# THU-luvision/TextureFusion

Hardware: AMD Instinct MI355X
Metric: RGB-D frames/s (TSDF integrate + atlas update: prepare->integrate->finalize, UpdateMeshes, GeneratePatches + UpdateAtlas over the frame's dirty chunks) (higher is better)
Workload: dtype f32

## Files before the change

texturefusion_amd/csrc/tf_mesh.hip:

```cpp
#include <stdlib.h>
#include <string.h>

#include <algorithm>
#include <vector>

#include "tf_devfn.h"
#include "tf_kf_store.h"
#include "tf_mc_table.h"
#include "tf_patch_body.h"
#include "tf_volume.h"

#pragma clang fp contract(off)

namespace tf {

__device__ const unsigned long long d_mc_tri[256] = TF_MC_TRI_TABLE_INIT;

constexpr int kR = 11;
constexpr int kRS = 11;
constexpr int kPS = kRS * kR;
constexpr int kRV = kPS * kR;
constexpr int kEdgeSlots = 3 * 729;
__device__ __forceinline__ uint32_t mesh_shard_rows_d(uint32_t max_chunks) { return max_chunks / kMeshShards + 258u; }

__device__ __forceinline__ int ridx(int x, int y, int z) { return (x + 1) + (y + 1) * kRS + (z + 1) * kPS; }

constexpr bool halo_needed(int rx, int ry, int rz) {
  if (rx < -1 || rx > 9 || ry < -1 || ry > 9 || rz < -1 || rz > 9) return false;
  if (rx >= 0 && rx < 8 && ry >= 0 && ry < 8 && rz >= 0 && rz < 8) return false;
  const int out = ((rx < 0 || rx > 8) ? 1 : 0) + ((ry < 0 || ry > 8) ? 1 : 0) + ((rz < 0 || rz > 8) ? 1 : 0);
  return out <= 1;
}
constexpr int count_halo_pairs() {
  int n = 0;
  for (int rz = -1; rz <= 9; ++rz)
    for (int ry = -1; ry <= 9; ++ry)
      for (int rx = -1; rx <= 9; ++rx) {
        if (!halo_needed(rx, ry, rz)) continue;
        const int vx = (rx + 8) & 7;
        if ((vx & 1) && halo_needed(rx - 1, ry, rz) && (((rx - 1 + 8) >> 3) == ((rx + 8) >> 3))) continue;
        ++n;
      }
  return n;
}
constexpr int kHalo = count_halo_pairs();
struct MeshTabs {
  unsigned long long halo[kHalo];
  uint16_t corner[729];
};
constexpr unsigned long long corner_of(int rx, int ry, int rz) {
  return (rx >= 0 && ry >= 0 && rz >= 0 && rx <= 8 && ry <= 8 && rz <= 8) ? (unsigned long long)(rx + ry * 9 + rz * 81 + 1) : 0ull;
}
constexpr MeshTabs make_mesh_tabs() {
  MeshTabs t{};
  int n = 0;
  for (int rz = -1; rz <= 9; ++rz)
    for (int ry = -1; ry <= 9; ++ry)
      for (int rx = -1; rx <= 9; ++rx) {
        if (!halo_needed(rx, ry, rz)) continue;
        const int vx = (rx + 8) & 7;
        const bool same_chunk_left = ((rx - 1 + 8) >> 3) == ((rx + 8) >> 3);
        if ((vx & 1) && halo_needed(rx - 1, ry, rz) && same_chunk_left) continue;
        const int rx0 = (vx & 1) ? rx - 1 : rx;
        const bool use0 = !(vx & 1);
        const bool use1 = (vx & 1) ? true : (halo_needed(rx + 1, ry, rz) && (((rx + 1 + 8) >> 3) == ((rx + 8) >> 3)));
        const int cx = (rx + 8) >> 3, cy = (ry + 8) >> 3, cz = (rz + 8) >> 3;
        const unsigned long long nb = (unsigned long long)(cx + cy * 3 + cz * 9);
        const unsigned long long pair = (unsigned long long)((((rx0 + 8) & 7) + ((ry + 8) & 7) * 8 + ((rz + 8) & 7) * 64) >> 1);
        const unsigned long long r0 = (unsigned long long)((rx0 + 1) + (ry + 1) * kRS + (rz + 1) * kPS);
        t.halo[n++] = (r0 & 2047ull) | (nb << 11) | (pair << 16) | ((use0 ? 1ull : 0ull) << 24) | ((use1 ? 1ull : 0ull) << 25) |
                      ((use0 ? corner_of(rx0, ry, rz) : 0ull) << 26) | ((use1 ? corner_of(rx0 + 1, ry, rz) : 0ull) << 36);
      }
  for (int c = 0; c < 729; ++c) {
    const int px = c % 9, py = (c / 9) % 9, pz = c / 81;
    t.corner[c] = (uint16_t)((px + 1) + (py + 1) * kRS + (pz + 1) * kPS);
  }
  return t;
}
__device__ const MeshTabs d_mesh_tabs = make_mesh_tabs();

__device__ __forceinline__ int cox(int k) { return (0x66 >> k) & 1; }
__device__ __forceinline__ int coy(int k) { return (0xCC >> k) & 1; }
__device__ __forceinline__ int coz(int k) { return (0xF0 >> k) & 1; }
__device__ __forceinline__ int edge_c0(int e) { return (int)((0x321076543210ull >> (4 * e)) & 0xF); }
__device__ __forceinline__ int edge_c1(int e) { return (int)((0x765447650321ull >> (4 * e)) & 0xF); }

__device__ __forceinline__ int edge_slot(int x, int y, int z, int e) {
  const int bx = x + ((0x622 >> e) & 1);
  const int by = y + ((0xC44 >> e) & 1);
  const int bz = z + ((0x0F0 >> e) & 1);
  const int ax = e >= 8 ? 2 : (e & 1);
  return ax + (bx + by * 9 + bz * 81) * 3;
}
__device__ __forceinline__ int edge_of_slot(int ax, int dx, int dy, int dz) {
  if (ax == 0) return dz ? (dy ? 6 : 4) : (dy ? 2 : 0);
  if (ax == 1) return dz ? (dx ? 5 : 7) : (dx ? 1 : 3);
  return dy ? (dx ? 10 : 11) : (dx ? 9 : 8);
}

__device__ __forceinline__ bool gradient_at(const float* __restrict__ S, int px, int py, int pz, int ox, int oy,
                                            int oz, float res, float g[3]) {
  const int c = ridx(px, py, pz);
  const float xm = S[c - 1], xp = S[c + 1];
  const float ym = S[c - kRS], yp = S[c + kRS];
  const float zm = S[c - kPS], zp = S[c + kPS];
  const bool ok = ((ox ? xp : xm) < 1.0f) && ((oy ? yp : ym) < 1.0f) && ((oz ? zp : zm) < 1.0f);
  const float gx = xp - xm, gy = yp - ym, gz = zp - zm;
  const float yz = gy * gy + gz * gz;
  const float sq = gx * gx + yz;
  const float n = sqrtf(sq);
  g[0] = gx; g[1] = gy; g[2] = gz;
  if (sq > 0.0f) { g[0] = gx / n; g[1] = gy / n; g[2] = gz / n; }
  return ok && !(n > res * 100.0f);
}

constexpr uint32_t kCfHeavy = 64u;
constexpr uint32_t kCfGradOk = 128u;

template <int NT>
struct MeshSh {
  float S[kRV];
  uint8_t cflag[732];
  uint32_t nslot[27];
  unsigned long long rmask[NT];
  uint16_t rbase[NT];
  uint32_t ownq[(kEdgeSlots + 7) / 8];
  uint16_t cinfo[512];
  uint8_t cidx[512];
  uint16_t toff[512];
  uint32_t wsum[8];
  uint32_t nv, nt, adj, any;
  uint32_t ncell;
  uint16_t clist[512];
  uint32_t ovf;
  uint32_t rblock;
  uint32_t rpress;
  uint32_t rstate;
  unsigned long long rtexloc;
};

__device__ __forceinline__ int edge_q(int e) {
  return (int)((0x231023320110ull >> (4 * e)) & 0x3);
}
__device__ __forceinline__ int owner_cell(int m, int q) {
  const int ax = m % 3, b = m / 3;
  const int bx = b % 9, by = (b / 9) % 9, bz = b / 81;
  const int d0 = q & 1, d1 = q >> 1;
  int x, y, z;
  if (ax == 0) { x = bx; y = by - d0; z = bz - d1; }
  else if (ax == 1) { x = bx - d0; y = by; z = bz - d1; }
  else { x = bx - d0; y = by - d1; z = bz; }
  return x + 8 * y + 64 * z;
}

__device__ __forceinline__ void patch_list_append(const VolumeDev& v, int ppar, uint32_t shard, const int4 id,
                                                  uint32_t slot, unsigned long long texloc, uint32_t blk) {
  const uint32_t rows = mesh_shard_rows_d(v.max_chunks);
  const uint32_t p = atomicAdd(&v.patch_cnt[((ppar & 1) * kMeshShards + shard) * 16], 1u);
  const unsigned long long key = pack_id(id.x, id.y, id.z);
  if (p < rows) v.patch_list[((size_t)(ppar & 1) * kMeshShards + shard) * rows + p] = make_int4((int)(uint32_t)key, (int)(uint32_t)(key >> 32), (int)slot, (int)blk);
  else atomicOr(&v.vctl->status, kStMeshFull);
  if (texloc == kNoTexloc) {
    const uint32_t c = atomicAdd(&v.actl->set[ppar & 1].n_cand, 1u);
    if (c < v.max_chunks) v.cand[c] = pack_id(id.x, id.y, id.z);
  }
}

__device__ __forceinline__ void filter_reset_record(const VolumeDev& v, uint32_t own, const int4 id, uint32_t epoch, int ppar) {
  MeshRec* rec = &v.mesh_rec[own];
  const uint32_t was = rec->state;
  const uint32_t inmap = was & kMsInMap;
  rec->nv = 0; rec->nt = 0; rec->state = inmap | ((ppar >= 0 && inmap) ? kMsSimplified : 0u); rec->epoch = epoch;
  if (inmap) {
    uint32_t blk = rec->block;
    const unsigned long long texloc = rec->texloc;
    if (blk != kBlkNone && blk_pressed(blk_pressure(v), blk)) {
      blk_release(v, blk);
      rec->block = blk = kBlkNone;
    }
    if (ppar >= 0) patch_list_append(v, ppar, own & (kMeshShards - 1u), id, own, texloc, blk);
  }
}

__device__ __forceinline__ void filter_defer_reset(const VolumeDev& v, uint32_t* cnt, uint32_t cap_sh, uint32_t own, const int4 id) {
  const uint32_t shard = own & (kMeshShards - 1u);
  const uint32_t p = atomicAdd(&cnt[(2u * kMeshShards + shard) * 16u], 1u);
  if (p < cap_sh) v.reset_list[(size_t)shard * cap_sh + p] = make_int4(id.x, id.y, id.z, (int)own);
}

__device__ const uint8_t kFarWord[19] = {0, 1, 2, 3, 4, 5, 6, 7, 8, 9, 10, 11, 12, 15, 18, 19, 20, 21, 24};
__device__ __forceinline__ uint32_t filter_near(const VolumeDev& v, const int4 id, int lane, int k8, uint32_t own_in, bool listed,
                                                bool use_summ, uint32_t create_seq, uint32_t* own, bool* maybe) {
  uint32_t nslot = kInvalidSlot;
  *maybe = true;
  if (own_in != kInvalidSlot) {
    const int word = k8 == 0 ? kNbrStamp : 13 + (k8 & 1) + 3 * ((k8 >> 1) & 1) + 9 * (k8 >> 2);
    uint32_t w = v.nbr[(size_t)own_in * kNbrWords + word];
    uint32_t alive = 1u;
    if (k8 == 0 && listed && id.w > 0) alive = v.hent[(uint32_t)id.w - 1u].alive & 1u;
    const uint32_t st = (uint32_t)__shfl((int)w, lane & 56);
    if (!(st > create_seq)) {
      if (k8 != 0 && w == 0u) {
        w = nbr_probe(v, pack_id(id.x + (k8 & 1), id.y + ((k8 >> 1) & 1), id.z + (k8 >> 2)));
        if (w) v.nbr[(size_t)own_in * kNbrWords + word] = w;
      }
      for (int q = k8; q < 19; q += 8) {
        const int fw = (int)kFarWord[q];
        if (v.nbr[(size_t)own_in * kNbrWords + fw] == 0u) {
          const uint32_t got = nbr_probe(v, pack_id(id.x + fw % 3 - 1, id.y + (fw / 3) % 3 - 1, id.z + fw / 9 - 1));
          if (got) v.nbr[(size_t)own_in * kNbrWords + fw] = got;
        }
      }
      if (k8 == 0) v.nbr[(size_t)own_in * kNbrWords + kNbrStamp] = v.seq;
    }
    nslot = k8 == 0 ? (alive ? own_in : kInvalidSlot) : (w ? w - 1u : kInvalidSlot);
  }
  *own = (uint32_t)__shfl((int)nslot, lane & 56);
  if (use_summ && *own != kInvalidSlot) {
    const uint32_t sm = nslot != kInvalidSlot ? v.summ[nslot] : 0u;
    const uint32_t sel = k8 == 0 ? 0u : ((k8 & 1) ? 4u : ((k8 & 2) ? 8u : 12u));
    uint32_t u = (sm >> sel) & 15u;
    u |= (uint32_t)__shfl_xor((int)u, 1); u |= (uint32_t)__shfl_xor((int)u, 2); u |= (uint32_t)__shfl_xor((int)u, 4);
    const uint32_t so = (uint32_t)__shfl((int)sm, lane & 56);
    *maybe = (so & 1u) && (u & 14u) == 14u;
  }
  return nslot;
}

template <bool HAVE_ROW>
__device__ __forceinline__ void filter_exact(const VolumeDev& v, const int4 id, uint32_t nslot, const uint32_t own, int lane,
                                             uint32_t epoch, uint32_t* __restrict__ surv, uint32_t* __restrict__ cnt,
                                             uint32_t cap_sh, int ppar, bool use_summ, bool defer, uint32_t create_seq) {
  const uint32_t shard = own & (kMeshShards - 1u);
  const float4* T4 = reinterpret_cast<const float4*>(v.tsdf + (size_t)own * kChunkVoxels);
  uint32_t roww = 0u;
  if (!HAVE_ROW && lane < kNbrWords) roww = v.nbr[(size_t)own * kNbrWords + lane];
  float4 qv[4];
#pragma unroll
  for (int j = 0; j < 4; ++j) qv[j] = T4[j * 64 + lane];
  const uint32_t had_mesh = v.mesh_rec[own].state & kMsInMap;
  uint32_t fl = 0;
#pragma unroll
  for (int j = 0; j < 4; ++j) {
    const float4 q = qv[j];
    const uint32_t c0 = classify_voxel(q.x, q.y), c1 = classify_voxel(q.z, q.w);
    fl |= c0 | c1 | ((lane & 3) ? 0u : c0 << 4) | ((lane & 28) ? 0u : (c0 | c1) << 8) | ((j || lane >= 32) ? 0u : (c0 | c1) << 12);
  }
  fl = wave_or(fl);
  if (!HAVE_ROW) {
    roww = nbr_row_checked(v, own, id, lane, roww, create_seq);
    nslot = lane == 13 ? own : ((lane < 27 && roww) ? roww - 1u : kInvalidSlot);
  }
  if (use_summ && lane == 0) v.summ[own] = fl;
  if (lane == 0) atomicAdd(&cnt[(kMeshShards + shard) * 16], 1u);
  bool empty = !(fl & 1u);
  if (!empty && (fl & 14u) != 14u) {
    uint32_t f2 = 0;
#pragma unroll
    for (int j = 0; j < 4; ++j) {
      const int q = j * 64 + lane;
      int cx = 0, cy = 0, cz = 0;
      if (q < 64) { cx = 8; cy = q & 7; cz = q >> 3; }
      else if (q < 128) { cx = q & 7; cy = 8; cz = (q >> 3) & 7; }
      else if (q < 192) { cx = q & 7; cy = (q >> 3) & 7; cz = 8; }
      else if (q < 200) { cx = 8; cy = 8; cz = q & 7; }
      else if (q < 208) { cx = 8; cy = q & 7; cz = 8; }
      else if (q < 216) { cx = q & 7; cy = 8; cz = 8; }
      else { cx = 8; cy = 8; cz = 8; }
      const uint32_t s = (uint32_t)__shfl((int)nslot, 13 + (cx >> 3) + 3 * (cy >> 3) + 9 * (cz >> 3));
      if (q < 217 && s != kInvalidSlot) {
        const float2 val = v.tsdf[(size_t)s * kChunkVoxels + (cx & 7) + (cy & 7) * 8 + (cz & 7) * 64];
        f2 |= classify_voxel(val.x, val.y);
      }
    }
    f2 = wave_or(f2);
    empty = ((fl | f2) & 14u) != 14u;
  }
  if (empty) {
    if (lane == 0) { if (defer) filter_defer_reset(v, cnt, cap_sh, own, id); else filter_reset_record(v, own, id, epoch, ppar); }
    return;
  }
  const bool back = !had_mesh;
  uint32_t p = 0;
  if (lane == 0) p = atomicAdd(&cnt[shard * 16 + (back ? 1 : 0)], 1u);
  p = (uint32_t)__builtin_amdgcn_readfirstlane((int)p);
  if (p >= cap_sh) {
    if (lane == 0) atomicOr(&v.vctl->status, kStMeshFull);
    return;
  }
  if (back) p = cap_sh - 1u - p;
  if (lane >= 27 && lane < 30) nslot = (uint32_t)(lane == 27 ? id.x : (lane == 28 ? id.y : id.z));
  if (lane < 30) surv[32 * ((size_t)shard * cap_sh + p) + lane] = nslot;
// ... 121 lines not shown
    for (uint32_t entry = wave; entry < n_flat; entry += nwaves) {
      const int4 id = dlist[entry];
      uint32_t own_listed = kInvalidSlot;
      if (dslot) own_listed = dslot[entry];
      process(id, own_listed, dslot != nullptr);
    }
    return;
  }
  __shared__ uint32_t s_n, s_ne;
  __shared__ uint32_t s_incl[kMeshShards], s_cnt[kMeshShards];
  if (threadIdx.x < kMeshShards) { s_incl[threadIdx.x] = sh_incl; s_cnt[threadIdx.x] = sh_n; }
  __shared__ uint32_t s_eown[32];
  __shared__ int4 s_eid[32];
  __shared__ int4 s_id[32];
  __shared__ uint32_t s_own[32];
  const int grp = threadIdx.x >> 3, k8 = threadIdx.x & 7;
  const uint32_t per = (n + nblk - 1) / nblk;
  const uint32_t first = bid * per;
  const uint32_t last = first + per < n ? first + per : n;
  for (uint32_t base = first; base < last; base += 32u) {
    if (threadIdx.x == 0) { s_n = 0; s_ne = 0; }
    __syncthreads();
    const uint32_t entry = base + (uint32_t)grp;
    if (entry < last) {
      int4 id;
      uint32_t own_in = kInvalidSlot;
      if (entry < n_flat) {
        id = dlist[entry];
        own_in = dslot ? dslot[entry] : hash_slot_alive(v, pack_id(id.x, id.y, id.z));
      } else {
        const uint32_t r = entry - n_flat;
        uint32_t shd = 0;
        for (uint32_t q = 0; q < kMeshShards; ++q) shd += s_incl[q] <= r ? 1u : 0u;
        shd &= kMeshShards - 1u;
        const size_t at = wl_base + (size_t)shd * wl_rows + (r - (s_incl[shd] - s_cnt[shd]));
        id = v.wl_ids[at];
        own_in = v.wl_slot[at];
      }
      uint32_t own;
      bool maybe;
      filter_near(v, id, lane, k8, own_in, dslot != nullptr || entry >= n_flat, use_summ, create_seq, &own, &maybe);
      if (fp.cls && ((fp.cls == 1u) != part_interior(v, id.x, id.y, id.z))) own = kInvalidSlot;
      if (own != kInvalidSlot && k8 == 0) {
        if (maybe) {
          const uint32_t at = atomicAdd(&s_n, 1u);
          s_own[at] = own; s_id[at] = id;
        } else {
          const uint32_t at = atomicAdd(&s_ne, 1u);
          s_eown[at] = own; s_eid[at] = id;
        }
      }
    }
    __syncthreads();
    if (w == 3 && lane < (int)s_ne) {
      if (fp.defer) filter_defer_reset(v, cnt, cap_sh, s_eown[lane], s_eid[lane]);
      else filter_reset_record(v, s_eown[lane], s_eid[lane], epoch, ppar);
    }
    const uint32_t nm = s_n;
    for (uint32_t m = (uint32_t)w; m < nm; m += 4u)
      filter_exact<false>(v, s_id[m], kInvalidSlot, s_own[m], lane, epoch, surv, cnt, cap_sh, ppar, use_summ, fp.defer != 0, create_seq);
    __syncthreads();
  }
}

__device__ __forceinline__ void mesh_stamp(const VolumeDev& v, uint32_t r, int k) {
  if (threadIdx.x == 0 && blockIdx.x < (uint32_t)kPhaseWaves && r == blockIdx.x)
    v.phase_buf[blockIdx.x * 16 + k] = __builtin_amdgcn_s_memrealtime();
}

#ifndef TF_MESH_WAVES
#define TF_MESH_WAVES 6
#endif
template <int NT, bool DBG = false>
__global__ __launch_bounds__(NT, TF_MESH_WAVES) void k_mesh(VolumeDev v, const uint32_t* __restrict__ surv, uint32_t* __restrict__ cnt,
                                                 uint32_t* __restrict__ cnt_next, uint32_t cap_sh,
                                                 uint32_t epoch, float res, uint32_t simplified, uint32_t dbg,
                                                 int rearm) {
  __shared__ MeshSh<NT> sh;
  extern __shared__ uint16_t vlist[];
  const int t = threadIdx.x, lane = t & 63;
  uint32_t n_rows = 0, excl_l = 0, incl_l = 0;
  {
    uint32_t my_n = cnt[(lane & 31) * 16 + (lane >> 5)];
    if (my_n > cap_sh) my_n = cap_sh;
    uint32_t incl = my_n;
#pragma unroll
    for (int o = 1; o < 64; o <<= 1) {
      const uint32_t u = (uint32_t)__shfl_up((int)incl, o);
      if (lane >= o) incl += u;
    }
    n_rows = (uint32_t)__builtin_amdgcn_readfirstlane(__shfl((int)incl, 63));
    const uint32_t r0 = blockIdx.x;
    const uint32_t sh0 = (uint32_t)__popcll(__ballot(incl <= r0));
    incl_l = (uint32_t)__builtin_amdgcn_readfirstlane(__shfl((int)incl, (int)(sh0 & 63u)));
    excl_l = incl_l - (uint32_t)__builtin_amdgcn_readfirstlane(__shfl((int)my_n, (int)(sh0 & 63u)));
    incl_l = (uint32_t)__builtin_amdgcn_readfirstlane((int)sh0);
  }
  if (blockIdx.x == 0 && t < (int)kMeshShards) { cnt_next[t * 16] = 0u; cnt_next[t * 16 + 1] = 0u; cnt_next[(kMeshShards + t) * 16] = 0u; cnt_next[(kMeshShards + t) * 16 + 1] = 0u; cnt_next[(2 * kMeshShards + t) * 16] = 0u; }
  if (blockIdx.x < kMeshShards) {
    uint32_t n_reset = cnt[(2u * kMeshShards + blockIdx.x) * 16u];
    if (n_reset > cap_sh) n_reset = cap_sh;
    for (uint32_t i = (uint32_t)t; i < n_reset; i += NT) {
      const int4 e = v.reset_list[(size_t)blockIdx.x * cap_sh + i];
      filter_reset_record(v, (uint32_t)e.w, make_int4(e.x, e.y, e.z, 0), epoch, rearm >= 0 ? (rearm ^ 1) : -1);
    }
  }
  const float half = res * 0.5f;
  if (rearm >= 0 && blockIdx.x == 0 && t == 0) {
    AtlasCtl::Set* O = &v.actl->set[rearm];
    O->n_work = 0; O->n_cand = 0; O->n_patch = 0; O->slots_base = 0ull;
    v.actl->set[rearm ^ 1].slots_base = v.actl->n_slots;
  }
  if (rearm >= 0 && blockIdx.x == 0 && t < (int)kMeshShards) {
    v.patch_cnt[((rearm & 1) * kMeshShards + t) * 16] = 0u;
    v.wl_cnt[((rearm & 1) * kMeshShards + t) * 16] = 0u;
  }
  if (DBG && dbg == 9) mesh_stamp(v, blockIdx.x, 0);
  for (uint32_t r = blockIdx.x; r < n_rows; r += gridDim.x) {
    uint32_t shard, own;
    int4 id;
    float2 a[512 / NT];
    {
      shard = incl_l;
      uint32_t idx = r - excl_l;
      if (r != blockIdx.x) {
        uint32_t my_n = cnt[(lane & 31) * 16 + (lane >> 5)];
        if (my_n > cap_sh) my_n = cap_sh;
        uint32_t incl = my_n;
#pragma unroll
        for (int o = 1; o < 64; o <<= 1) {
          const uint32_t u = (uint32_t)__shfl_up((int)incl, o);
          if (lane >= o) incl += u;
        }
        shard = (uint32_t)__builtin_amdgcn_readfirstlane((int)__popcll(__ballot(incl <= r)));
        idx = r - (uint32_t)__builtin_amdgcn_readfirstlane(__shfl((int)incl, (int)(shard & 63u)) - __shfl((int)my_n, (int)(shard & 63u)));
      }
      if (shard >= kMeshShards) { shard -= kMeshShards; idx = cap_sh - 1u - idx; }
      const size_t row = (size_t)shard * cap_sh + idx;
      own = surv[32 * row + 13];
      id = make_int4((int)surv[32 * row + 27], (int)surv[32 * row + 28], (int)surv[32 * row + 29], 0);
#pragma unroll
      for (int j = 0; j < 512 / NT; ++j) a[j] = v.tsdf[(size_t)own * kChunkVoxels + j * NT + t];
      __syncthreads();
      if (t < 27) sh.nslot[t] = surv[32 * row + t];
    }
    int t_ = threadIdx.x;
    asm volatile("" : "+v"(t_));
    const int t = t_, lane = t & 63, w = t >> 6;
    MeshRec* rec = &v.mesh_rec[own];
    unsigned long long htab[(kHalo + NT - 1) / NT];
#pragma unroll
    for (int j = 0; j < (kHalo + NT - 1) / NT; ++j) htab[j] = (j * NT + t < kHalo) ? d_mesh_tabs.halo[j * NT + t] : ~0ull;
    if (DBG && dbg == 9) mesh_stamp(v, r, 1);
    if (t == 0) { sh.nv = 0; sh.nt = 0; sh.adj = 0; sh.ncell = 0; }
    if (t == NT - 64) { sh.rstate = rec->state; sh.rblock = rec->block; sh.rtexloc = rec->texloc; sh.rpress = blk_pressure(v); }
    if (DBG && dbg == 1) continue;
#pragma unroll
    for (int j = 0; j < 512 / NT; ++j) {
      const int q = j * NT + t;
      const int x0 = q & 7, y0 = (q >> 3) & 7, z0 = q >> 6;
      sh.S[ridx(x0, y0, z0)] = a[j].x; sh.cflag[x0 + y0 * 9 + z0 * 81] = (a[j].y > 50.0f) ? kCfHeavy : 0u;
    }
    __syncthreads();
#pragma unroll
    for (int j = 0; j < (kHalo + NT - 1) / NT; ++j) {
      const unsigned long long e = htab[j];
      if (e == ~0ull) continue;
      const uint32_t s = sh.nslot[(uint32_t)(e >> 11) & 31u];
      float4 val = make_float4(999.0f, 0.0f, 999.0f, 0.0f);
      if (s != kInvalidSlot) val = reinterpret_cast<const float4*>(v.tsdf + (size_t)s * kChunkVoxels)[(uint32_t)(e >> 16) & 255u];
      const uint32_t r0 = (uint32_t)e & 2047u;
      if ((e >> 24) & 1ull) {
        sh.S[r0] = val.x;
        const uint32_t cf = (uint32_t)(e >> 26) & 1023u;
        if (cf) sh.cflag[cf - 1u] = (val.y > 50.0f) ? kCfHeavy : 0u;
      }
      if ((e >> 25) & 1ull) {
        sh.S[r0 + 1u] = val.z;
        const uint32_t cf = (uint32_t)(e >> 36) & 1023u;
        if (cf) sh.cflag[cf - 1u] = (val.w > 50.0f) ? kCfHeavy : 0u;
      }
    }
    __syncthreads();
    if (DBG && dbg == 9) mesh_stamp(v, r, 3);
    for (int c = t; c < 729; c += NT) {
      const int r = d_mesh_tabs.corner[c];
      const float xm = sh.S[r - 1], xp = sh.S[r + 1], ym = sh.S[r - kRS], yp = sh.S[r + kRS];
      const float zm = sh.S[r - kPS], zp = sh.S[r + kPS];
      uint32_t f = (xm < 1.0f ? 1u : 0u) | (xp < 1.0f ? 2u : 0u) | (ym < 1.0f ? 4u : 0u) | (yp < 1.0f ? 8u : 0u) |
                   (zm < 1.0f ? 16u : 0u) | (zp < 1.0f ? 32u : 0u);
      const float gx = xp - xm, gy = yp - ym, gz = zp - zm;
      const float yz = gy * gy + gz * gz;
      const float nrm = sqrtf(gx * gx + yz);
      if (!(nrm > res * 100.0f)) f |= kCfGradOk;
      sh.cflag[c] |= (uint8_t)f;
    }
    for (int i = t; i < (kEdgeSlots + 7) / 8; i += NT) sh.ownq[i] = 0u;
    __syncthreads();

    if (DBG && dbg == 2) continue;
    if (DBG && dbg == 9) mesh_stamp(v, r, 4);
    for (int cell = t; cell < 512; cell += NT) {
      const int x = cell & 7, y = (cell >> 3) & 7, z = cell >> 6;
      const int c0 = ridx(x, y, z);
      bool observed = true;
      int pos = 0, index = 0;
#pragma unroll
      for (int k = 0; k < 8; ++k) {
        const float s = sh.S[c0 + cox(k) + coy(k) * kRS + coz(k) * kPS];
        observed = observed && !(s > 1.0f);
        pos += (s > 0.0f) ? 1 : 0;
        index |= (0.0f > s) ? (1 << k) : 0;
      }
      sh.cinfo[cell] = 0;
      if (observed && (pos % 8) > 0 && index != 0 && index != 255)
        sh.clist[atomicAdd(&sh.ncell, 1u)] = (uint16_t)cell;
    }
    __syncthreads();
    if (t == 0 && sh.ncell) atomicAdd(&cnt[(kMeshShards + shard) * 16 + 1], 1u);
    for (uint32_t ci = t; ci < sh.ncell; ci += NT) {
      const int cell = sh.clist[ci];
      const int x = cell & 7, y = (cell >> 3) & 7, z = cell >> 6;
      const int c0 = ridx(x, y, z);
      float cube[8];
      int index = 0;
#pragma unroll
      for (int k = 0; k < 8; ++k) {
        const float s = sh.S[c0 + cox(k) + coy(k) * kRS + coz(k) * kPS];
        cube[k] = s;
        index |= (0.0f > s) ? (1 << k) : 0;
      }
      const unsigned long long row = d_mc_tri[index];
      uint32_t valid = 0;
      const int cf0 = x + y * 9 + z * 81;
#pragma unroll
      for (int e = 0; e < 12; ++e) {
        const int e0 = (int)((0x321076543210ull >> (4 * e)) & 0xF), e1 = (int)((0x765447650321ull >> (4 * e)) & 0xF);
        const float s0 = cube[e0], s1 = cube[e1];
        const bool far = fabsf(s0) > fabsf(s1);
        const int ko = far ? (cox(e1) + coy(e1) * 9 + coz(e1) * 81) : (cox(e0) + coy(e0) * 9 + coz(e0) * 81);
        const uint32_t need0 = kCfHeavy | kCfGradOk | (1u << cox(e0)) | (4u << coy(e0)) | (16u << coz(e0));
        const uint32_t need1 = kCfHeavy | kCfGradOk | (1u << cox(e1)) | (4u << coy(e1)) | (16u << coz(e1));
        const uint32_t need = far ? need1 : need0;
        if (s0 * s1 < 0.0f) {
          const uint32_t have = sh.cflag[cf0 + ko];
          if ((have & need) == need) valid |= 1u << e;
        }
      }
      uint32_t ntri = 0, used = 0;
#pragma unroll 1
      for (int col = 0; col < 15; col += 3) {
        const int s0 = (int)((row >> (4 * col)) & 0xF);
        if (s0 == 0xF) break;
        const int s1 = (int)((row >> (4 * col + 4)) & 0xF), s2 = (int)((row >> (4 * col + 8)) & 0xF);
        if (!((valid >> s0) & (valid >> s1) & (valid >> s2) & 1u)) continue;
        ++ntri;
        used |= (1u << s0) | (1u << s1) | (1u << s2);
      }
      for (uint32_t u = used; u; u &= u - 1) {
        const int e = __builtin_ctz(u);
        const int m = edge_slot(x, y, z, e);
        atomicOr(&sh.ownq[m >> 3], 1u << (4 * (m & 7) + edge_q(e)));
      }
      sh.cinfo[cell] = (uint16_t)(used | (ntri << 12));
      sh.cidx[cell] = (uint8_t)index;
    }
    __syncthreads();

    if (DBG && dbg == 3) continue;
    if (DBG && dbg == 9) mesh_stamp(v, r, 5);
    {
      constexpr int kEpt = 2304 / NT, kCpt = 512 / NT;
      const int first = t * kEpt;
      unsigned long long usedm = 0;
      {
        constexpr int kWords = (kEpt * 4 + 31) / 32 + 1;
        const int w0 = first >> 3, sh0 = 4 * (first & 7);
#pragma unroll
        for (int q = 0; q < kWords; ++q) {
          const int wi = w0 + q;
          uint32_t x = wi < (kEdgeSlots + 7) / 8 ? sh.ownq[wi] : 0u;
          x |= x >> 1; x |= x >> 2; x &= 0x11111111u;
          x = (x | (x >> 3)) & 0x03030303u;
          x = (x | (x >> 6)) & 0x000F000Fu;
          x = (x | (x >> 12)) & 0xFFu;
          usedm |= (unsigned long long)x << (8 * q);
        }
        usedm >>= (sh0 >> 2);
        usedm &= (1ull << kEpt) - 1ull;
        const int left = kEdgeSlots - first;
        if (left < kEpt) usedm = left > 0 ? (usedm & ((1ull << left) - 1ull)) : 0ull;
      }
      const uint32_t cnt = (uint32_t)__popcll(usedm);
      uint32_t tc = 0;
#pragma unroll
      for (int j = 0; j < kCpt; ++j) tc += (uint32_t)sh.cinfo[kCpt * t + j] >> 12;
      uint32_t pk = cnt | (tc << 16);
      uint32_t inc = pk;
#pragma unroll
      for (int o = 1; o < 64; o <<= 1) {
        const uint32_t u = __shfl_up(inc, o);
        if (lane >= o) inc += u;
      }
      if (lane == 63) sh.wsum[w] = inc;
      __syncthreads();
      uint32_t before = 0, total = 0;
      for (int k = 0; k < NT / 64; ++k) {
        if (k < w) before += sh.wsum[k];
        total += sh.wsum[k];
      }
      if (t == 0) sh.ovf = mesh_block_for(v, sh.rblock, total & 0xFFFFu, total >> 16, sh.rpress);
      __syncthreads();
      const uint32_t ovf_blk = sh.ovf;
      uint16_t* const gvl = (ovf_blk != kBlkFail && (ovf_blk & kBlkLarge)) ? v.ovf_vlist + (size_t)((ovf_blk & ~kBlkLarge) - 1u) * kOvfCV : nullptr;
      const uint32_t excl = before + inc - pk;
      uint32_t r = excl & 0xFFFFu;
      sh.rbase[t] = (uint16_t)r;
      sh.rmask[t] = usedm;
      for (unsigned long long u = usedm; u; u &= u - 1ull) {
        const int m = first + (int)__builtin_ctzll(u);
        if (gvl) { if (r < (uint32_t)kOvfCV) gvl[r] = (uint16_t)m; }
        else if (r < v.mesh_cv) vlist[r] = (uint16_t)m;
        ++r;
      }
      uint32_t t0 = excl >> 16;
#pragma unroll
      for (int j = 0; j < kCpt; ++j) {
        sh.toff[kCpt * t + j] = (uint16_t)t0;
        t0 += (uint32_t)sh.cinfo[kCpt * t + j] >> 12;
      }
      if (t == 0) { sh.nv = total & 0xFFFFu; sh.nt = total >> 16; }
    }
    __syncthreads();
    const uint32_t nv = sh.nv, nt = sh.nt;
    const uint32_t ovf = sh.ovf;
    if (ovf == kBlkFail) {
      if (t == 0) {
        atomicOr(&v.vctl->status, kStMeshFull);
        const uint32_t was = sh.rstate & kMsInMap;
        rec->nv = 0; rec->nt = 0; rec->state = was | kMsOverflow; rec->epoch = epoch;
        if (rearm >= 0 && was) patch_list_append(v, rearm ^ 1, shard, id, own, sh.rtexloc, sh.rblock);
      }
      __syncthreads();
      continue;
    }
    const uint16_t* const gvlist = (ovf & kBlkLarge) ? v.ovf_vlist + (size_t)((ovf & ~kBlkLarge) - 1u) * kOvfCV : nullptr;

    if (DBG && dbg == 4) continue;
    if (DBG && dbg == 9) mesh_stamp(v, r, 6);
    const uint32_t inmap = (sh.rstate & kMsInMap) | (nv ? kMsInMap : 0u);
    if (t == NT - 64) {
      mesh_block_settle(v, sh.rblock, ovf);
      if (rearm >= 0 && inmap) patch_list_append(v, rearm ^ 1, shard, id, own, sh.rtexloc, ovf);
    }
    const float org[3] = {(float)(8 * id.x) * res, (float)(8 * id.y) * res, (float)(8 * id.z) * res};
    uint32_t adj = 0;
    for (uint32_t i = t; i < nv; i += NT) {
      const int m = gvlist ? gvlist[i] : vlist[i];
      const int cell = owner_cell(m, __builtin_ctz((sh.ownq[m >> 3] >> (4 * (m & 7))) & 0xFu));
      const int x = cell & 7, y = (cell >> 3) & 7, z = cell >> 6;
      const int ax = m % 3, b = m / 3;
      const int bx = b % 9, by = (b / 9) % 9, bz = b / 81;
      const int e = edge_of_slot(ax, bx - x, by - y, bz - z);
      const int e0 = edge_c0(e), e1 = edge_c1(e);
      const float s0 = sh.S[ridx(x + cox(e0), y + coy(e0), z + coz(e0))];
      const float s1 = sh.S[ridx(x + cox(e1), y + coy(e1), z + coz(e1))];
      const float tt = s0 / (s0 - s1);
      const int o0[3] = {cox(e0), coy(e0), coz(e0)}, o1[3] = {cox(e1), coy(e1), coz(e1)};
      const int cc[3] = {x, y, z};
      float pv[3];
#pragma unroll
      for (int a = 0; a < 3; ++a) {
        const float p0 = (float)o0[a] * res, p1 = (float)o1[a] * res;
        const float ev = p0 + tt * (p1 - p0);
        const float origin = org[a] + ((float)cc[a] * res + half);
        pv[a] = ev + origin;
      }
      const int k = (fabsf(s0) > fabsf(s1)) ? e1 : e0;
      const int px = x + cox(k), py = y + coy(k), pz = z + coz(k);
      float g[3];
      gradient_at(sh.S, px, py, pz, cox(k), coy(k), coz(k), res, g);
      const uint32_t cs = sh.nslot[((px + 8) >> 3) + ((py + 8) >> 3) * 3 + ((pz + 8) >> 3) * 9];
      const ushort4 c4 = v.color[(size_t)cs * kChunkVoxels + (px & 7) + (py & 7) * 8 + (pz & 7) * 64];
      float col[3] = {1.0f, 1.0f, 1.0f};
      const float cw = (float)c4.w;
      if (cw > 0.0f) {
        col[0] = ((float)c4.x / 255.0f) / cw;
        col[1] = ((float)c4.y / 255.0f) / cw;
        col[2] = ((float)c4.z / 255.0f) / cw;
      }
#pragma unroll
      for (int a = 0; a < 3; ++a) {
        mesh_plane(v, ovf, kMpPos + a)[i] = pv[a];
        mesh_plane(v, ovf, kMpNrm + a)[i] = g[a];
        mesh_plane(v, ovf, kMpCol + a)[i] = col[a];
        const int gp = (int)floorf((pv[a] - org[a]) / (res * 1.0f));
        if (gp >= 8) adj |= 1u << (2 * a + 1);
        if (gp <= 0) adj |= 1u << (2 * a);
      }
    }
    if (adj) atomicOr(&sh.adj, adj);
    if (DBG && dbg == 9) mesh_stamp(v, r, 7);
    for (uint32_t ci = (uint32_t)(NT - 1 - t); ci < sh.ncell; ci += NT) {
      const int cell = sh.clist[ci];
      const uint32_t info = sh.cinfo[cell];
      if (!(info >> 12)) continue;
      const int x = cell & 7, y = (cell >> 3) & 7, z = cell >> 6;
      const unsigned long long row = d_mc_tri[sh.cidx[cell]];
      const uint32_t valid = info & 0xFFFu;
      uint32_t o = sh.toff[cell];
      for (int col = 0; col < 15; col += 3) {
        const int s0 = (int)((row >> (4 * col)) & 0xF);
        if (s0 == 0xF) break;
        const int s1 = (int)((row >> (4 * col + 4)) & 0xF), s2 = (int)((row >> (4 * col + 8)) & 0xF);
        if (!((valid >> s0) & (valid >> s1) & (valid >> s2) & 1u)) continue;
        constexpr int kEptT = 2304 / NT;
        auto ref_of = [&](int m) {
          const int tt = m / kEptT, j = m - tt * kEptT;
          return (uint16_t)(sh.rbase[tt] + (uint32_t)__popcll(sh.rmask[tt] & ((1ull << j) - 1ull)));
        };
        tri_plane(v, ovf, 0)[o] = ref_of(edge_slot(x, y, z, s2));
        tri_plane(v, ovf, 1)[o] = ref_of(edge_slot(x, y, z, s1));
        tri_plane(v, ovf, 2)[o] = ref_of(edge_slot(x, y, z, s0));
        ++o;
      }
    }
    __syncthreads();
    if (t == 0) {
      rec->nv = (uint16_t)nv; rec->nt = (uint16_t)nt; rec->epoch = epoch; rec->block = ovf;
      rec->state = inmap | (sh.adj << kMsAdjShift) | (inmap ? simplified : 0u);
    }
    __syncthreads();
    if (DBG && dbg == 9) mesh_stamp(v, r, 8);
  }
}

__global__ __launch_bounds__(256) void k_init_mesh_rec(MeshRec* rec, uint32_t n) {
  for (uint32_t i = blockIdx.x * 256 + threadIdx.x; i < n; i += gridDim.x * 256) {
    MeshRec r;
    memset(&r, 0, sizeof(r));
    r.texloc = kNoTexloc;
    r.frameid = -1;
    r.ratio[0] = r.ratio[1] = 1.0f;
    rec[i] = r;
  }
}
void launch_init_meshes(const VolumeDev& v, hipStream_t s) {
  hipLaunchKernelGGL(k_init_mesh_rec, dim3(1024), dim3(256), 0, s, v.mesh_rec, v.max_chunks);
  (void)hipMemsetAsync(v.mesh_rec + v.max_chunks, 0, sizeof(uint32_t) * ((size_t)blk_ring_len(v.mesh_blocks) + blk_ring_len(v.ovf_blocks)), s);
  (void)hipMemsetAsync(v.mesh_cnt, 0, sizeof(uint32_t) * 2 * kMeshCntWords, s);
}

uint32_t mesh_shard_rows(uint32_t max_chunks) { return max_chunks / kMeshShards + 258u; }

static void launch_mesher(const VolumeDev& v, int cnt_par, uint32_t max_entries, uint32_t epoch, float res, bool fused,
                          int rearm_set, hipStream_t s) {
  static const uint32_t dbg = getenv("TF_MESH_DBG") ? (uint32_t)atoi(getenv("TF_MESH_DBG")) : 0u;
  uint32_t* surv = v.mesh_nbr;
  uint32_t* cnt = v.mesh_cnt + (size_t)(cnt_par & 1) * kMeshCntWords;
  uint32_t* cnt_next = v.mesh_cnt + (size_t)((cnt_par & 1) ^ 1) * kMeshCntWords;
  const uint32_t cap_sh = mesh_shard_rows(v.max_chunks);
  uint32_t grid = ((max_entries + kMeshShards - 1) / kMeshShards + 1) * kMeshShards;
  static const uint32_t gmax = (uint32_t)device_cus() * (uint32_t)(TF_MESH_WAVES * 2);
  if (grid > gmax) grid = gmax;
  if (dbg)
    hipLaunchKernelGGL((k_mesh<128, true>), dim3(grid), dim3(128), v.mesh_cv * sizeof(uint16_t), s, v, surv, cnt, cnt_next, cap_sh, epoch, res,
                       fused ? kMsSimplified : 0u, dbg, rearm_set);
  else
    hipLaunchKernelGGL((k_mesh<128>), dim3(grid), dim3(128), v.mesh_cv * sizeof(uint16_t), s, v, surv, cnt, cnt_next, cap_sh, epoch, res,
                       fused ? kMsSimplified : 0u, 0u, rearm_set);
}

bool launch_mesh(const VolumeDev& v, int cnt_par, const int4* dlist, const uint32_t* dcount, uint32_t max_entries,
                 uint32_t epoch, float res, bool fused, int rearm_set, uint32_t len_guess, uint32_t* len_hint, int shards_par,
                 hipStream_t s, const PatchStage* patch, const Cam* cam, int cls, const KfStoreArgs* store) {
  if (!max_entries) return false;
  uint32_t* cnt = v.mesh_cnt + (size_t)(cnt_par & 1) * kMeshCntWords;
  const uint32_t cap_sh = mesh_shard_rows(v.max_chunks);
  if (max_entries > v.max_chunks) max_entries = v.max_chunks;
  const uint32_t fmax = 2560u;
  const uint32_t fgrid = (max_entries + 3) / 4 < fmax ? (max_entries + 3) / 4 : fmax;
  const uint32_t* dslot = fused ? v.work_slot : nullptr;
  const int ppar = fused ? (rearm_set ^ 1) : -1;
  const bool use_summ = true;
  const bool wave_form = len_guess <= 2560u * 4u;
  FilterPatch fp;
  memset(&fp, 0, sizeof(fp));
  fp.cls = (uint32_t)cls;
  if (store) { fp.n_store = 1u; fp.store = *store; }
  if (patch && cam) {
    fp.defer = 1u;
    fp.n_patch = 1024u;
    fp.first = 0u;
    fp.par = patch->par;
    fp.cam = *cam;
    fp.kf = patch->kf;
  }
#define TF_LAUNCH_FILTER(W, P)                                                                                       \
  hipLaunchKernelGGL((k_mesh_filter<W, P>), dim3(fgrid + fp.n_patch + fp.n_store), dim3(256), 0, s, v, dlist, dslot, dcount, max_entries, \
                     epoch, v.mesh_nbr, cnt, cap_sh, ppar, use_summ, len_hint, shards_par, fp)
  static const bool tl = getenv("TF_MESH_DBG") && atoi(getenv("TF_MESH_DBG")) == 10;
  if (wave_form && tl && !fp.n_patch)
    hipLaunchKernelGGL((k_mesh_filter<true, false, true>), dim3(fgrid + fp.n_store), dim3(256), 0, s, v, dlist, dslot, dcount, max_entries,
                       epoch, v.mesh_nbr, cnt, cap_sh, ppar, use_summ, len_hint, shards_par, fp);
  else if (wave_form) { if (fp.n_patch) TF_LAUNCH_FILTER(true, true); else TF_LAUNCH_FILTER(true, false); }
  else { if (fp.n_patch) TF_LAUNCH_FILTER(false, true); else TF_LAUNCH_FILTER(false, false); }
#undef TF_LAUNCH_FILTER
  launch_mesher(v, cnt_par, max_entries, epoch, res, fused, rearm_set, s);
  return fp.n_patch != 0;
}

constexpr uint32_t kDirtyBlocks = 512;
__device__ __forceinline__ void dirty_frame_body(const VolumeDev& v, int par, uint32_t stamp) {
  const SelBuf& L = v.sel;
  const uint32_t nl = L.ctl->n_list <= v.max_list ? L.ctl->n_list : 0u;
  const uint32_t total = nl * 8u;
  AtlasCtl::Set* S = &v.actl->set[par];
  const int lane = threadIdx.x & 63, w = threadIdx.x >> 6;
  __shared__ uint32_t wcnt[16];
  __shared__ uint32_t gbase;
  for (uint32_t b0 = blockIdx.x * 1024; b0 < total; b0 += kDirtyBlocks * 1024) {
    const uint32_t t = b0 + threadIdx.x;
    bool emit = false;
    int4 q = make_int4(0, 0, 0, 0);
    uint32_t slot = kInvalidSlot;
    if (t < total && (t & 7u) != 7u) {
      const uint32_t e = list_phys(v, t >> 3, L.ctl->n_front);
      const int k = (int)(t & 7u);
      const int4 id0 = L.list_id[e];
      const uint32_t slot0 = L.list_slot[e];
      if (L.list_needs[e]) {
        q = nbr7(id0, k);
        q.w = 0;
        if (k == 0) slot = slot0;
        else slot = hash_slot_alive(v, pack_id(q.x, q.y, q.z));
        if (slot != kInvalidSlot && part_owned(v, q.x, q.y, q.z))
          emit = atomicMax(&v.mesh_rec[slot].stamp, stamp) < stamp;
      }
    }
    const unsigned long long m = __ballot(emit);
    if (lane == 0) wcnt[w] = (uint32_t)__popcll(m);
    __syncthreads();
    if (threadIdx.x == 0) {
      uint32_t tot = 0;
      for (int k = 0; k < 16; ++k) { const uint32_t c = wcnt[k]; wcnt[k] = tot; tot += c; }
      gbase = tot ? atomicAdd(&S->n_work, tot) : 0u;
    }
    __syncthreads();
    if (emit) {
      const uint32_t p = gbase + wcnt[w] + (uint32_t)__popcll(m & ((1ull << lane) - 1ull));
      if (p < v.max_chunks) { v.work_ids[p] = q; v.work_slot[p] = slot; }
    }
    __syncthreads();
  }
}
__global__ __launch_bounds__(1024) void k_dirty_frame(VolumeDev v, int par, uint32_t stamp) { dirty_frame_body(v, par, stamp); }
__global__ __launch_bounds__(1024) void k_dirty_frame_store(VolumeDev v, int par, uint32_t stamp, KfStoreArgs a) {
  if (blockIdx.x == kDirtyBlocks) { kf_store_body(v, a.tab, a.slots, a.arena, a.cap, a.slot, a.slack, a.fill); return; }
  dirty_frame_body(v, par, stamp);
}
void launch_dirty_frame(const VolumeDev& v, int par, uint32_t stamp, hipStream_t s) {
  hipLaunchKernelGGL(k_dirty_frame, dim3(kDirtyBlocks), dim3(1024), 0, s, v, par, stamp);
}
void launch_dirty_frame_store(const VolumeDev& v, int par, uint32_t stamp, const KfStoreArgs& a, hipStream_t s) {
  hipLaunchKernelGGL(k_dirty_frame_store, dim3(kDirtyBlocks + 1), dim3(1024), 0, s, v, par, stamp, a);
}

__global__ __launch_bounds__(256) void k_adopt_dirty_list(VolumeDev v, int par) {
  uint32_t n = v.vctl->n_tmp;
  if (n > v.max_chunks) n = v.max_chunks;
  if (blockIdx.x == 0 && threadIdx.x == 0) v.actl->set[par].n_work = n;
  for (uint32_t i = blockIdx.x * 256 + threadIdx.x; i < n; i += gridDim.x * 256) {
// ... 416 lines not shown
```

Before: 10760.

## Classify surface cells with bitmask rows and compute corner flags only where needed

Replaces the per-cell eight-corner classification with per-row bitmasks over the 9x9x9 corner grid. Surface cells are found by OR-ing four rows and shifting, and corner gradient flags are then computed only for corners that touch a surface cell, not for all 729. The new scratch tables share shared memory with the ranking tables through a union, which keeps the LDS footprint unchanged. It adds two extra barriers, and the classification of corner flags for unneeded corners changes, which is only safe if nothing downstream reads those corners.

```diff
diff --git a/texturefusion_amd/csrc/tf_mesh.hip b/texturefusion_amd/csrc/tf_mesh.hip
--- a/texturefusion_amd/csrc/tf_mesh.hip
+++ b/texturefusion_amd/csrc/tf_mesh.hip
@@ -46,7 +46,6 @@
 constexpr int kHalo = count_halo_pairs();
 struct MeshTabs {
   unsigned long long halo[kHalo];
-  uint16_t corner[729];
 };
 constexpr unsigned long long corner_of(int rx, int ry, int rz) {
   return (rx >= 0 && ry >= 0 && rz >= 0 && rx <= 8 && ry <= 8 && rz <= 8) ? (unsigned long long)(rx + ry * 9 + rz * 81 + 1) : 0ull;
@@ -71,10 +70,6 @@
         t.halo[n++] = (r0 & 2047ull) | (nb << 11) | (pair << 16) | ((use0 ? 1ull : 0ull) << 24) | ((use1 ? 1ull : 0ull) << 25) |
                       ((use0 ? corner_of(rx0, ry, rz) : 0ull) << 26) | ((use1 ? corner_of(rx0 + 1, ry, rz) : 0ull) << 36);
       }
-  for (int c = 0; c < 729; ++c) {
-    const int px = c % 9, py = (c / 9) % 9, pz = c / 81;
-    t.corner[c] = (uint16_t)((px + 1) + (py + 1) * kRS + (pz + 1) * kPS);
-  }
   return t;
 }
 __device__ const MeshTabs d_mesh_tabs = make_mesh_tabs();
@@ -122,12 +117,24 @@
   float S[kRV];
   uint8_t cflag[732];
   uint32_t nslot[27];
-  unsigned long long rmask[NT];
-  uint16_t rbase[NT];
+  struct Rank {
+    unsigned long long rmask[NT];
+    uint16_t rbase[NT];
+    uint16_t toff[512];
+  };
+  struct Front {
+    uint16_t nlist[736];
+    uint32_t cmask[81];
+    uint8_t lrow[64];
+  };
+  union {
+    Rank rk;
+    Front fr;
+  };
   uint32_t ownq[(kEdgeSlots + 7) / 8];
-  uint16_t cinfo[512];
+  alignas(8) uint16_t cinfo[512];
   uint8_t cidx[512];
-  uint16_t toff[512];
+  uint32_t nneed;
   uint32_t wsum[8];
   uint32_t nv, nt, adj, any;
   uint32_t ncell;
@@ -138,6 +145,7 @@
   uint32_t rstate;
   unsigned long long rtexloc;
 };
+static_assert(sizeof(MeshSh<128>::Front) <= sizeof(MeshSh<128>::Rank), "the front tables live in the ranking tables' storage");
 
 __device__ __forceinline__ int edge_q(int e) {
   return (int)((0x231023320110ull >> (4 * e)) & 0x3);
@@ -565,7 +573,7 @@
 #pragma unroll
     for (int j = 0; j < (kHalo + NT - 1) / NT; ++j) htab[j] = (j * NT + t < kHalo) ? d_mesh_tabs.halo[j * NT + t] : ~0ull;
     if (DBG && dbg == 9) mesh_stamp(v, r, 1);
-    if (t == 0) { sh.nv = 0; sh.nt = 0; sh.adj = 0; sh.ncell = 0; }
+    if (t == 0) { sh.nv = 0; sh.nt = 0; sh.adj = 0; sh.ncell = 0; sh.nneed = 0; }
     if (t == NT - 64) { sh.rstate = rec->state; sh.rblock = rec->block; sh.rtexloc = rec->texloc; sh.rpress = blk_pressure(v); }
     if (DBG && dbg == 1) continue;
 #pragma unroll
@@ -596,8 +604,51 @@
     }
     __syncthreads();
     if (DBG && dbg == 9) mesh_stamp(v, r, 3);
-    for (int c = t; c < 729; c += NT) {
-      const int r = d_mesh_tabs.corner[c];
+    if (t < 81) {
+      const int py = t % 9, pz = t / 9;
+      const float* const row = &sh.S[ridx(0, py, pz)];
+      uint32_t m = 0;
+#pragma unroll
+      for (int i = 0; i < 9; ++i) {
+        const float s = row[i];
+        m |= ((s > 1.0f) ? (1u << i) : 0u) | ((s > 0.0f) ? (1u << (9 + i)) : 0u) | ((0.0f > s) ? (1u << (18 + i)) : 0u);
+      }
+      sh.fr.cmask[t] = m;
+    }
+    for (int i = t; i < (kEdgeSlots + 7) / 8; i += NT) sh.ownq[i] = 0u;
+    for (int i = t; i < 512 / 4; i += NT) reinterpret_cast<unsigned long long*>(sh.cinfo)[i] = 0ull;
+    __syncthreads();
+    if (t < 64) {
+      const int cr = (t & 7) + 9 * (t >> 3);
+      uint32_t A = sh.fr.cmask[cr] | sh.fr.cmask[cr + 1] | sh.fr.cmask[cr + 9] | sh.fr.cmask[cr + 10];
+      A |= A >> 1;
+      const uint32_t l = ~A & (A >> 9) & (A >> 18) & 0xFFu;
+      sh.fr.lrow[t] = (uint8_t)l;
+      if (l) {
+        uint32_t at = atomicAdd(&sh.ncell, (uint32_t)__popc(l));
+        for (uint32_t u = l; u; u &= u - 1u) sh.clist[at++] = (uint16_t)(8 * t + __builtin_ctz(u));
+      }
+    }
+    __syncthreads();
+    if (t == 0 && sh.ncell) atomicAdd(&cnt[(kMeshShards + shard) * 16 + 1], 1u);
+    if (t < 81) {
+      const int py = t % 9, pz = t / 9;
+      uint32_t l = 0;
+      if (py < 8 && pz < 8) l |= sh.fr.lrow[py + 8 * pz];
+      if (py > 0 && pz < 8) l |= sh.fr.lrow[py - 1 + 8 * pz];
+      if (py < 8 && pz > 0) l |= sh.fr.lrow[py + 8 * (pz - 1)];
+      if (py > 0 && pz > 0) l |= sh.fr.lrow[py - 1 + 8 * (pz - 1)];
+      const uint32_t need = l | (l << 1);
+      if (need) {
+        uint32_t at = atomicAdd(&sh.nneed, (uint32_t)__popc(need));
+        for (uint32_t u = need; u; u &= u - 1u) sh.fr.nlist[at++] = (uint16_t)(__builtin_ctz(u) | (py << 4) | (pz << 8));
+      }
+    }
+    __syncthreads();
+    for (uint32_t i = t; i < sh.nneed; i += NT) {
+      const uint32_t e = sh.fr.nlist[i];
+      const int px = (int)(e & 15u), py = (int)((e >> 4) & 15u), pz = (int)(e >> 8);
+      const int r = ridx(px, py, pz);
       const float xm = sh.S[r - 1], xp = sh.S[r + 1], ym = sh.S[r - kRS], yp = sh.S[r + kRS];
       const float zm = sh.S[r - kPS], zp = sh.S[r + kPS];
       uint32_t f = (xm < 1.0f ? 1u : 0u) | (xp < 1.0f ? 2u : 0u) | (ym < 1.0f ? 4u : 0u) | (yp < 1.0f ? 8u : 0u) |
@@ -606,31 +657,12 @@
       const float yz = gy * gy + gz * gz;
       const float nrm = sqrtf(gx * gx + yz);
       if (!(nrm > res * 100.0f)) f |= kCfGradOk;
-      sh.cflag[c] |= (uint8_t)f;
-    }
-    for (int i = t; i < (kEdgeSlots + 7) / 8; i += NT) sh.ownq[i] = 0u;
+      sh.cflag[px + py * 9 + pz * 81] |= (uint8_t)f;
+    }
     __syncthreads();
 
     if (DBG && dbg == 2) continue;
     if (DBG && dbg == 9) mesh_stamp(v, r, 4);
-    for (int cell = t; cell < 512; cell += NT) {
-      const int x = cell & 7, y = (cell >> 3) & 7, z = cell >> 6;
-      const int c0 = ridx(x, y, z);
-      bool observed = true;
-      int pos = 0, index = 0;
-#pragma unroll
-      for (int k = 0; k < 8; ++k) {
-        const float s = sh.S[c0 + cox(k) + coy(k) * kRS + coz(k) * kPS];
-        observed = observed && !(s > 1.0f);
-        pos += (s > 0.0f) ? 1 : 0;
-        index |= (0.0f > s) ? (1 << k) : 0;
-      }
-      sh.cinfo[cell] = 0;
-      if (observed && (pos % 8) > 0 && index != 0 && index != 255)
-        sh.clist[atomicAdd(&sh.ncell, 1u)] = (uint16_t)cell;
-    }
-    __syncthreads();
-    if (t == 0 && sh.ncell) atomicAdd(&cnt[(kMeshShards + shard) * 16 + 1], 1u);
     for (uint32_t ci = t; ci < sh.ncell; ci += NT) {
       const int cell = sh.clist[ci];
       const int x = cell & 7, y = (cell >> 3) & 7, z = cell >> 6;
@@ -728,8 +760,8 @@
       uint16_t* const gvl = (ovf_blk != kBlkFail && (ovf_blk & kBlkLarge)) ? v.ovf_vlist + (size_t)((ovf_blk & ~kBlkLarge) - 1u) * kOvfCV : nullptr;
       const uint32_t excl = before + inc - pk;
       uint32_t r = excl & 0xFFFFu;
-      sh.rbase[t] = (uint16_t)r;
-      sh.rmask[t] = usedm;
+      sh.rk.rbase[t] = (uint16_t)r;
+      sh.rk.rmask[t] = usedm;
       for (unsigned long long u = usedm; u; u &= u - 1ull) {
         const int m = first + (int)__builtin_ctzll(u);
         if (gvl) { if (r < (uint32_t)kOvfCV) gvl[r] = (uint16_t)m; }
@@ -739,7 +771,7 @@
       uint32_t t0 = excl >> 16;
 #pragma unroll
       for (int j = 0; j < kCpt; ++j) {
-        sh.toff[kCpt * t + j] = (uint16_t)t0;
+        sh.rk.toff[kCpt * t + j] = (uint16_t)t0;
         t0 += (uint32_t)sh.cinfo[kCpt * t + j] >> 12;
       }
       if (t == 0) { sh.nv = total & 0xFFFFu; sh.nt = total >> 16; }
@@ -821,7 +853,7 @@
       const int x = cell & 7, y = (cell >> 3) & 7, z = cell >> 6;
       const unsigned long long row = d_mc_tri[sh.cidx[cell]];
       const uint32_t valid = info & 0xFFFu;
-      uint32_t o = sh.toff[cell];
+      uint32_t o = sh.rk.toff[cell];
       for (int col = 0; col < 15; col += 3) {
         const int s0 = (int)((row >> (4 * col)) & 0xF);
         if (s0 == 0xF) break;
@@ -830,7 +862,7 @@
         constexpr int kEptT = 2304 / NT;
         auto ref_of = [&](int m) {
           const int tt = m / kEptT, j = m - tt * kEptT;
-          return (uint16_t)(sh.rbase[tt] + (uint32_t)__popcll(sh.rmask[tt] & ((1ull << j) - 1ull)));
+          return (uint16_t)(sh.rk.rbase[tt] + (uint32_t)__popcll(sh.rk.rmask[tt] & ((1ull << j) - 1ull)));
         };
         tri_plane(v, ovf, 0)[o] = ref_of(edge_slot(x, y, z, s2));
         tri_plane(v, ovf, 1)[o] = ref_of(edge_slot(x, y, z, s1));
```

Result: slower. 10410 (-3.3%).
